# Gyeeta/gyeeta

Measured on AMD Instinct MI355X. Metric: events/sec ingested + p50/p99 quantile error vs reference, 1→8 MI355X, higher is better.
Workload: dtype int64; 1 GPU; C3/C4: 10000 hosts x 1000 services, raw 24-B tcp_ipv4_resp_event_t stream, uniform over services, 1 window (ingest + window close) per step; service_keys_total=10000000, multi_level_windows=0, td_pend_cap=1920, td_pend_cap_is_library_default=False, exchange=none, exchange_requested=none, exchange_fallback=False

## Files before the change

gyeeta_amd/capi.py:

```python
import ctypes as C
import os

HERE = os.path.dirname(os.path.abspath(__file__))
LIB_PATH = os.environ.get("GYS_LIB") or os.path.join(HERE, "lib", "libgysketch.so")

OK, ERR_INVAL, ERR_NOMEM, ERR_HIP, ERR_NOTFOUND, ERR_NOT_OWNER, ERR_STATE, ERR_INTERNAL = 0, -1, -2, -3, -4, -5, -6, -7
MAX_BUCKETS, TD_NB, HLL_P, CMS_D, CMS_W, NSTATES, TOPN = 16, 200, 14, 4, 65536, 6, 10
NLEVELS, LEVEL_RING = 4, 10
TD_PEND_CAP = 896
RCCL_UID_BYTES = 128
KINDS = {"RESP_TIME_HASH": 0, "SEMI_LOG_HASH": 1, "SEMI_LOG_HASH_LO": 2, "DURATION_HASH": 3, "HASH_10_5000": 4, "HASH_5_250": 5,
         "HASH_1_3000": 6, "PERCENT_HASH": 7}


class Config(C.Structure):
    _fields_ = [("struct_size", C.c_uint32), ("device", C.c_int32), ("rank", C.c_uint32), ("nranks", C.c_uint32),
                ("max_hosts", C.c_uint32), ("max_services", C.c_uint32), ("max_clusters", C.c_uint32),
                ("enable_tdigest", C.c_uint32), ("svc_hll_p", C.c_uint32), ("resp_path", C.c_uint32),
                ("max_batch_events", C.c_uint64), ("stream", C.c_void_p), ("reduce_arena", C.c_void_p),
                ("reduce_arena_bytes", C.c_uint64), ("enable_levels", C.c_uint32), ("td_buf_values", C.c_uint32),
                ("conn_pair_cms", C.c_uint32), ("td_pend_cap", C.c_uint32), ("svc_hll_levels", C.c_uint32)]


class ListenerInfo(C.Structure):
# ... 210 lines not shown
    "gys_num_services": (C.c_uint32, [vp]),
    "gys_num_hosts": (C.c_uint32, [vp]),
    "gys_lookup_service": (C.c_int, [vp, C.c_uint64, u32p]),
    "gys_export_hist": (C.c_int, [vp, C.c_int, C.c_uint32, C.c_uint32, vp]),
    "gys_export_conn_bitmap": (C.c_int, [vp, C.c_uint32, C.c_uint32, vp]),
    "gys_export_hll": (C.c_int, [vp, vp]),
    "gys_export_cms": (C.c_int, [vp, C.c_int, vp]),
    "gys_export_tdigest": (C.c_int, [vp, C.c_uint32, C.c_uint32, vp, vp, vp]),
    "gys_export_tdigest_pending": (C.c_int, [vp, C.c_uint32, C.c_uint32, vp, vp]),
    "gys_export_svc_counters": (C.c_int, [vp, C.c_uint32, C.c_uint32, vp]),
    "gys_export_global_hist": (C.c_int, [vp, C.POINTER(HistRec)]),
    "gys_export_svc_hll": (C.c_int, [vp, C.c_uint32, C.c_uint32, vp]),
    "gys_export_svc_hll_level": (C.c_int, [vp, C.c_int, C.c_uint64, C.c_uint32, C.c_uint32, vp]),
    "gys_get_counters": (C.c_int, [vp, C.POINTER(Counters)]),
    "gys_resp_queue_pending": (C.c_int, [vp, u64p]),
    "gys_hist_init_dev": (C.c_int, [vp, C.c_int, vp, C.c_uint32]),
    "gys_hist_add_dev": (C.c_int, [vp, C.c_int, vp, C.c_uint32, vp, vp, C.c_uint64]),
    "gys_hist_merge_dev": (C.c_int, [vp, vp, vp, C.c_uint32]),
    "gys_hist_percentiles_dev": (C.c_int, [vp, C.c_int, vp, C.c_uint32, f32p, C.c_uint32, vp]),
    "gys_profile_enable": (C.c_int, [vp, C.c_int]),
    "gys_profile_reset": (C.c_int, [vp]),
    "gys_profile_get": (C.c_int, [vp, C.c_char_p, f64p, u64p]),
    "gys_profile_names": (C.c_int, [vp, C.c_char_p, C.c_size_t]),
    "gys_debug_read_events_dev": (C.c_int, [vp, vp, C.c_uint64]),
    "gys_gen_resp_events_dev": (C.c_int, [vp, vp, C.c_uint64, C.c_uint64, C.c_uint32, C.c_uint32, C.c_uint32, C.c_uint32, C.POINTER(RespSeg)]),
}

_lib = None


# ... 31 lines not shown
```

gyeeta_amd/csrc/gys_device.hpp:

```cpp
#pragma once

#include <hip/hip_runtime.h>
#include <stdint.h>

#include "../../include/gysketch.h"
#include "../../include/gys_tdigest_tbl.h"

#define GYS_WAVE 64
#ifndef GYS_OPAQUE_VGPR
#define GYS_OPAQUE_VGPR(x) asm volatile("" : "+v"(x))
#endif
#ifndef GYS_DYN_LDS
#define GYS_DYN_LDS(type, name) extern __shared__ type name[]
#endif
#define GYS_SEED 0xceedfeadu
#define GYS_GOLDEN 0x9e3779b9u
#define GYS_NOSLOT 0xFFFFFFFFu
#define GYS_EMPTY_KEY 0xFFFFFFFFFFFFFFFFull

#ifndef GYS_KERNARG
#define GYS_KERNARG 1
#endif
#if GYS_KERNARG && defined(__HIP_DEVICE_COMPILE__)
#define GYS_KERNARG_REF(T, name, arg)                                                             \
// ... 79 lines not shown
	b += (uint32_t)(key >> 32);
	a += (uint32_t)(key & 0xFFFFFFFFu);
	jmix(a, b, c);
	return c;
}

__host__ __device__ __forceinline__ uint32_t host_tbl_hash(uint32_t netns, uint32_t port)
{
	uint32_t x = netns ^ ((port & 0xFFFFu) * 0x9E3779u);
	x ^= x >> 16;
	return x * 0x85EBCA6Bu;
}
__host__ __device__ __forceinline__ uint32_t host_tbl_hash(uint64_t key48) { return host_tbl_hash((uint32_t)(key48 >> 16), (uint32_t)(key48 & 0xFFFFu)); }
__host__ __device__ __forceinline__ uint32_t host_tbl_slot(uint32_t hk, uint32_t mask) { return (hk ^ (hk >> 13)) & mask; }
__host__ __device__ __forceinline__ uint32_t host_tbl_part(uint32_t hk, uint32_t pmask) { return (hk >> 21) & pmask; }

struct HashDef {
	int32_t nthr;
	int32_t is_fixed_diff;
	int32_t arg_bits, t_bits;
	int64_t thr[14];
	int64_t fd_min, fd_maxp1, fd_diff;
};

#define GYS_HASH_DEFS_INIT                                                                                                  \
	{                                                                                                                   \
		{13, 0, 64, 64, {1, 10, 30, 60, 100, 150, 200, 300, 450, 700, 1000, 3000, 15000}, 0, 0, 0},                      \
		{12, 0, 32, 32, {1, 10, 100, 500, 1000, 5000, 25000, 50000, 100000, 300000, 1000000, 5000000}, 0, 0, 0},      \
		{13, 0, 32, 32, {1, 10, 50, 200, 500, 1000, 3000, 6000, 10000, 15000, 25000, 60000, 150000}, 0, 0, 0},        \
		{13, 0, 32, 32, {1, 10, 25, 50, 125, 400, 1000, 3000, 6000, 10000, 25000, 40000, 65000}, 0, 0, 0},            \
// ... 304 lines not shown
```

gyeeta_amd/csrc/gys_engine.hip:

```cpp
#include <hip/hip_runtime.h>

#include <algorithm>
#include <array>
#include <atomic>
#include <chrono>
#include <cmath>
#include <cstdarg>
#include <cstdio>
#include <cstdlib>
#include <cstring>
#include <deque>
#include <map>
#include <string>
#include <thread>
#include <condition_variable>
#include <mutex>
#include <unordered_map>
#include <unordered_set>
#include <vector>

#include <dlfcn.h>
#include <rccl/rccl.h>

#include "gys_kernels.hpp"
// ... 47 lines not shown
	memcpy(&m.first, id, 8);
	memcpy(&m.second, id + 8, 8);
	return m;
}

struct ProfEntry {
	double total_ms = 0;
	uint64_t launches = 0;
	std::vector<std::pair<hipEvent_t, hipEvent_t>> pending;
};

inline uint64_t align_up(uint64_t v, uint64_t a) { return (v + a - 1) / a * a; }

struct HostListeners {
	std::vector<uint64_t> tbl;
	std::vector<uint32_t> slots;
	std::vector<uint32_t> all_slots;
	std::vector<uint64_t> keys;
	uint32_t tbl_off = 0, tbl_cap = 0, lst_off = 0;
	bool on_device = false;
	bool overflow = false;
	std::vector<HostListeners> sub;
	uint32_t sub_desc = 0;
	struct LAddr {
		uint32_t ip32 = 0;
		uint32_t ip128[4] = {0, 0, 0, 0};
		bool any = true;
	};
	struct ChainEnt {
		uint32_t slot;
// ... 407 lines not shown
		set_err("host belongs to rank %u", gys_shard_of(machine_id, c->cfg.nranks));
		return GYS_ERR_NOT_OWNER;
	}
	return GYS_OK;
}

uint32_t next_pow2(uint64_t v)
{
	uint64_t p = 1;
	while (p < v) p <<= 1;
	return (uint32_t)p;
}

inline uint64_t host_key48(uint32_t netns, uint16_t port) { return ((uint64_t)netns << 16) | (uint64_t)port; }

int64_t host_tbl_find(const HostListeners &hl, uint64_t key48)
{
	if (hl.tbl.empty()) return -1;
	const uint32_t mask = (uint32_t)hl.tbl.size() - 1;
	uint32_t h = host_tbl_slot(host_tbl_hash(key48), mask);
	for (uint32_t probes = 0; probes <= mask; ++probes) {
		const uint64_t e = hl.tbl[h];
		if (e == GYS_HOST_TBL_EMPTY) return -1;
		if ((e >> 16) == key48) return (int64_t)h;
		h = (h + 1) & mask;
	}
	return -1;
}

void host_tbl_put(HostListeners &hl, uint64_t key48, uint32_t local)
{
	const uint32_t mask = (uint32_t)hl.tbl.size() - 1;
	uint32_t h = host_tbl_slot(host_tbl_hash(key48), mask);
	while (hl.tbl[h] != GYS_HOST_TBL_EMPTY) h = (h + 1) & mask;
	hl.tbl[h] = (key48 << 16) | (uint64_t)local;
}

inline uint32_t host_part_of(uint64_t key48, uint32_t nparts) { return host_tbl_part(host_tbl_hash(key48), nparts - 1u); }

#define GYS_HOST_TBL_SPARSE 4096u
inline uint32_t host_tbl_capacity(size_t n)
{
	static const uint32_t sparse = [] { const char *e = getenv("GYS_TBL_SPARSE"); return e ? (uint32_t)atoi(e) : GYS_HOST_TBL_SPARSE; }();
	const uint32_t c4 = next_pow2(std::max<uint64_t>(16, (uint64_t)n * 4));
	return c4 <= sparse ? c4 : std::max<uint32_t>(std::min<uint32_t>(sparse, c4), next_pow2(std::max<uint64_t>(16, (uint64_t)n * 2)));
}

int host_tbl_upload(gys_ctx *c, HostListeners &hl, uint32_t desc, uint32_t part, uint32_t nparts, uint32_t cand_off, bool *ok)
{
	*ok = true;
	if (!hl.on_device || hl.tbl.size() > hl.tbl_cap) {
		if (c->htbl_used + hl.tbl.size() > c->htbl_cap || c->hlst_used + hl.tbl.size() / 2 > c->hlst_cap) {
			*ok = false;
			return GYS_OK;
		}
		hl.tbl_off = (uint32_t)c->htbl_used;
		hl.tbl_cap = (uint32_t)hl.tbl.size();
		c->htbl_used += hl.tbl.size();
		hl.lst_off = (uint32_t)c->hlst_used;
		c->hlst_used += hl.tbl.size() / 2;
		hl.on_device = true;
	}
	HIPCHK(hipMemcpyAsync(c->htbl + hl.tbl_off, hl.tbl.data(), hl.tbl.size() * 8, hipMemcpyHostToDevice, c->stream));
	if (!hl.slots.empty()) HIPCHK(hipMemcpyAsync(c->hlst + hl.lst_off, hl.slots.data(), hl.slots.size() * 4, hipMemcpyHostToDevice, c->stream));
	const HostDesc hd{hl.tbl_off, (uint32_t)hl.tbl.size() - 1, (uint32_t)hl.slots.size(), hl.lst_off, part, nparts - 1u, cand_off, 0u};
	HIPCHK(hipMemcpyAsync(c->hdesc + desc, &hd, sizeof(hd), hipMemcpyHostToDevice, c->stream));
	HIPCHK(hipStreamSynchronize(c->stream));
	return GYS_OK;
}

int host_cands_upload(gys_ctx *c, HostListeners &hl)
{
	if (hl.cands.empty()) return GYS_OK;
	if (hl.cands.size() > hl.cand_cap) {
		const uint64_t want = std::max<uint64_t>(16, next_pow2(hl.cands.size()));
		const uint64_t bound = 4ull * c->cfg.max_services + 64ull * c->cfg.max_hosts;
		if (c->cand_used + want > bound) {
			set_err("listener candidate pool exhausted");
			return GYS_ERR_NOMEM;
		}
// ... 148 lines not shown

void host_rebind_local(HostListeners &hl, uint64_t key48, uint32_t slot, uint32_t new_slot)
{
	if (hl.overflow) return;
	HostListeners &t = hl.sub.empty() ? hl : hl.sub[host_part_of(key48, (uint32_t)hl.sub.size())];
	for (uint32_t l = 0; l < t.slots.size(); ++l)
		if (t.slots[l] == slot && t.keys[l] == key48) {
			t.slots[l] = new_slot;
			return;
		}
}

int host_lst_add(gys_ctx *c, uint32_t host, const gys_listener_info *arr, uint32_t n, uint32_t first_slot)
{
	HostListeners &hl = c->host_lst[host];
	auto new_local = [&](uint64_t key48, uint32_t slot) {
		if (hl.overflow) return false;
		HostListeners *t = hl.sub.empty() ? &hl : &hl.sub[host_part_of(key48, (uint32_t)hl.sub.size())];
		while (t->slots.size() >= GYS_HOST_MAX_LOCAL) {
			if (!host_lst_repartition(c, hl, hl.sub.empty() ? 2u : (uint32_t)hl.sub.size() * 2u)) {
				hl.overflow = true;
				auto take = [&](const HostListeners &s) {
					for (uint32_t l = 0; l < s.keys.size(); ++l)
						if (!hl.chain.count(s.keys[l])) hl.okey[s.keys[l]] = s.slots[l];
				};
				if (hl.sub.empty()) take(hl);
				else for (const HostListeners &s : hl.sub) take(s);
				return false;
			}
			t = &hl.sub[host_part_of(key48, (uint32_t)hl.sub.size())];
		}
		host_tbl_insert(hl, *t, key48, slot);
		return true;
	};
	for (uint32_t i = 0; i < n; ++i) {
		const uint64_t key48 = host_key48(arr[i].netns, arr[i].port);
		const uint32_t slot = first_slot + i;
		const HostListeners::LAddr a = listener_addr(arr[i]);
		auto ch = hl.chain.find(key48);
		if (ch != hl.chain.end()) {
			bool replaced = false;
			for (HostListeners::ChainEnt &e : ch->second) {
				if (e.a.any || laddr_equal(e.a, a)) {
					host_rebind_local(hl, key48, e.slot, slot);
					e.slot = slot;
					e.a = a;
					replaced = true;
// ... 24 lines not shown
			if (hl.overflow && a.any) hl.okey[key48] = slot;
		} else if (!hl.overflow) {
			new_local(key48, slot);
			if (hl.overflow && a.any) hl.okey[key48] = slot;
		} else if (a.any) {
			hl.okey[key48] = slot;
		}
		if (!a.any) {
			hl.okey.erase(key48);
			hl.chain[key48].push_back(HostListeners::ChainEnt{slot, a});
			hl.dirty = true;
		}
	}
	if (hl.dirty) {
		host_rebuild(hl);
		const int rc = host_cands_upload(c, hl);
		if (rc) return rc;
		std::vector<uint64_t> kv;
		for (const auto &cf : hl.cand_first) {
			kv.push_back(listener_key(host, (uint32_t)(cf.first >> 16), (uint16_t)(cf.first & 0xFFFFu)));
			kv.push_back((uint64_t)(GYS_SLOT_GROUP | (hl.cand_off + cf.second)));
		}
		if (!kv.empty()) {
			const uint32_t nk = (uint32_t)(kv.size() / 2);
			const int rs = ensure_staging(c, kv.size() * 8, 0);
			if (rs) return rs;
			HIPCHK(hipMemcpyAsync(c->dev_staging, kv.data(), kv.size() * 8, hipMemcpyHostToDevice, c->stream));
			hipLaunchKernelGGL(k_table_set, dim3((nk + 255) / 256), dim3(256), 0, c->stream, c->lk_tbl, (const uint64_t *)c->dev_staging, nk);
			HIPCHK(hipStreamSynchronize(c->stream));
		}
// ... 3531 lines not shown
	HLL_LEVEL_CHECK(level);
	if (!nslots) return GYS_OK;
	uint8_t *tmp = nullptr;
	HIPCHK(hipMalloc((void **)&tmp, (size_t)nslots << c->cfg.svc_hll_p));
	const int rc = hll_level_view(c, level, tusec, first_slot, nslots, tmp, nullptr);
	hipError_t e = hipSuccess;
	if (rc == GYS_OK) e = hipMemcpyAsync(out, tmp, (size_t)nslots << c->cfg.svc_hll_p, hipMemcpyDeviceToHost, c->stream);
	const hipError_t es = hipStreamSynchronize(c->stream);
	hipFree(tmp);
	if (rc) return rc;
	HIPCHK(e);
	HIPCHK(es);
	return GYS_OK;
} GYS_CATCH_ALL

int gys_get_counters(gys_ctx *c, gys_counters *out)
try {
	GYS_ENTER(c);
	if (!c || !out) return GYS_ERR_INVAL;
	uint64_t v[32];
	static_assert(CTR_NUM <= 31, "counter block (the last word is the sink of k_read_events)");
	HIPCHK(hipMemcpyAsync(v, c->counters, sizeof(v), hipMemcpyDeviceToHost, c->stream));
	HIPCHK(hipStreamSynchronize(c->stream));
#ifdef GYS_RESP_TIMING
	{
		unsigned long long t[16];
		HIPCHK(hipMemcpyFromSymbol(t, HIP_SYMBOL(gys::g_resp_timing), sizeof(t)));
		unsigned long long tot = 0;
		for (int i = 0; i < 12; ++i) tot += t[i];
		static const char *nm[12] = {"loads", "probe2", "probe3+", "kept/atomics", "ghist+hash", "hllq/store", "barrier1", "scan1+b", "scan2+b", "image+b", "prologue", "flush"};
// ... 426 lines not shown
```

gyeeta_amd/csrc/gys_kernels.hpp:

```cpp
#pragma once

#include "gys_device.hpp"

namespace gys {

#define GYS_HUGE_VALUE_BITS 20
#define GYS_HUGE_BINS (1u << GYS_HUGE_VALUE_BITS)
#define GYS_ROW_BITS 6
#define GYS_ROW_MASK 0x3Fu
#define GYS_ROW_V6 0x20u
#define GYS_BM_WORDS 32u
#define GYS_STAGED_WORD(tresp, cli_port) ((uint64_t)(((uint32_t)(tresp) << GYS_ROW_BITS) | ((uint32_t)(cli_port) & 0x1Fu)))
#define GYS_STAGED_WORD_FAM(tresp, cli_port, v6) ((uint32_t)(((uint32_t)(tresp) << GYS_ROW_BITS) | ((v6) ? GYS_ROW_V6 : 0u) | ((uint32_t)(cli_port) & 0x1Fu)))

enum { CTR_RESP_EVENTS = 0, CTR_RESP_DROP_RANGE, CTR_RESP_DROP_NOLISTENER, CTR_CONN_EVENTS, CTR_CONN_UNKNOWN, CTR_LSTATE_RECORDS,
       CTR_LSTATE_MISSED, CTR_LSTATE_ERRORS, CTR_LSTATE_DELETED, CTR_TD_MERGES, CTR_TD_MERGE_VALUES, CTR_ACTCONN_RECORDS, CTR_ACTCONN_REMOTE_LISTEN, CTR_ACTCONN_UNKNOWN,
       CTR_CONN_NEW, CTR_CONN_CLOSED, CTR_CONN_CLOSED_NO_NOTIFY, CTR_CONN_CLI_SIDE, CTR_RESP_RUN_OVERFLOW, CTR_NUM };

__global__ void k_table_insert(DevTable t, const uint64_t *keys, uint32_t first_val, uint32_t n, uint32_t *nfail)
{
	const uint32_t i = blockIdx.x * blockDim.x + threadIdx.x;
	if (i >= n) return;
	const uint64_t key = keys[i];
	uint32_t h = get_uint64_hash(key) & t.mask;
// ... 656 lines not shown
__global__ __launch_bounds__(256) void k_cms_reduce(const uint32_t *partial, uint32_t nch, uint32_t *cms32)
{
	const uint32_t i = blockIdx.x * blockDim.x + threadIdx.x;
	if (i >= GYS_CMS_D * GYS_CMS_W) return;
	uint32_t sum = 0;
	for (uint32_t c = 0; c < nch; ++c) sum += partial[(size_t)c * GYS_CMS_D * GYS_CMS_W + i];
	if (sum) cms32[i] += sum;
}

#ifndef GYS_BUCKET_LUT
#define GYS_BUCKET_LUT 1
#endif
#ifndef GYS_SHIFT_SWITCH
#define GYS_SHIFT_SWITCH 0
#endif
#ifndef GYS_PROBE_XOR
#define GYS_PROBE_XOR 1
#endif
#ifndef GYS_BK_BYTES
#define GYS_BK_BYTES 1
#endif
#ifndef GYS_PARK_INDEX
#define GYS_PARK_INDEX 1
#endif
#ifndef GYS_EV_DMA
#define GYS_EV_DMA 0
#endif
#ifndef GYS_EV_DMA_AHEAD
#define GYS_EV_DMA_AHEAD 1
#endif
#if defined(__HIP_DEVICE_COMPILE__)
#ifndef GYS_EV_DMA_CPOL
#define GYS_EV_DMA_CPOL 0
#endif
#define GYS_DMA16(gptr, ldsptr) __builtin_amdgcn_global_load_lds((const __attribute__((address_space(1))) void *)(gptr), (__attribute__((address_space(3))) void *)(ldsptr), 16, 0, GYS_EV_DMA_CPOL)
#define GYS_DMA_WAIT() asm volatile("s_waitcnt vmcnt(0)" ::: "memory")
#else
#define GYS_DMA16(gptr, ldsptr) memcpy((char *)(ldsptr) + 16u * (threadIdx.x & 63u), (const void *)(gptr), 16)
#define GYS_DMA_WAIT() ((void)0)
#endif
#ifndef GYS_EV_PREFETCH
#define GYS_EV_PREFETCH 0
#endif
#ifndef GYS_FLOOR_QUARTER
#define GYS_FLOOR_QUARTER 1
#endif
#ifndef GYS_HASH_FLAT
#define GYS_HASH_FLAT 1
#endif
#ifndef GYS_PROBE_JOINT
#define GYS_PROBE_JOINT 0
#endif
__device__ __forceinline__ void resp_bucket_lut_init(uint32_t *s_bk, uint32_t tid, uint32_t nthreads)
{
	for (uint32_t i = tid; i < 256u; i += nthreads)
		s_bk[i] = resp_bucket((int64_t)(4u * i)) | (resp_bucket((int64_t)(4u * i + 1u)) << 8) | (resp_bucket((int64_t)(4u * i + 2u)) << 16) |
			  (resp_bucket((int64_t)(4u * i + 3u)) << 24);
}
__device__ __forceinline__ uint32_t resp_bucket_lut(const uint32_t *s_bk, uint32_t tresp)
{
	if (!GYS_BUCKET_LUT) return resp_bucket((int64_t)tresp);
#if GYS_BK_BYTES
	uint32_t bix = tresp & 1023u;
#if defined(__HIP_DEVICE_COMPILE__)
	asm volatile("" : "+v"(bix));
#endif
// ... 1 lines not shown
#else
	const uint32_t lo = (s_bk[(tresp >> 2) & 255u] >> ((tresp & 3u) * 8u)) & 0xFFu;
#endif
	const uint32_t hi = 12u + (tresp > 3000u) + (tresp > 15000u);
	return tresp < 1024u ? lo : hi;
}

struct HostDesc {
	uint32_t tbl_off;
	uint32_t mask;
	uint32_t nlst;
	uint32_t lst_off;
	uint32_t part;
	uint32_t pmask;
	uint32_t cand_off;
	uint32_t pad;
};

#define GYS_HOST_TBL_EMPTY 0xFFFFFFFFFFFFFFFFull
#define GYS_EV_DROPPED 0xFFFFFFFFu
#define GYS_HOST_THREADS 1024
#define GYS_RESP_THREADS(TPT) (((TPT) == 12 || (TPT) == 32) ? 512 : 1024)
#define GYS_RESP_WAVES_PER_SIMD(TPT) ((TPT) == 32 ? 2 : 4)
#define GYS_SPLIT_PART 65536u

#ifdef GYS_RESP_TIMING
__device__ unsigned long long g_resp_timing[16];
#define GYS_TICK(i) do { const unsigned long long t_now__ = (unsigned long long)clock64(); tacc[i] += (uint32_t)(t_now__ - t_prev__); t_prev__ = t_now__; } while (0)
#else
#define GYS_TICK(i) do { } while (0)
#endif
struct RespHostP {
	const uint64_t *ev;
	uint64_t n;
// ... 12 lines not shown
	long long run_delta;
	uint32_t *staged;
	const uint32_t *host_spill;
	uint32_t spill_stamp;
	uint64_t *counters;
	uint8_t *svc_hll;
	uint32_t svc_hll_p;
	unsigned long long *ghist;
	long long *gmax;
	uint32_t lds_tbl_entries;
	uint32_t lds_key_entries;
	FinP fin;
	uint32_t dbg;
};

__host__ __device__ __forceinline__ size_t resp_host_lds_bytes(uint32_t tbl_entries, uint32_t key_entries, uint32_t tile)
{
	return ((size_t)tbl_entries + 2u) * 8u + (size_t)key_entries * 24u + ((size_t)tile + 2u) * 6u;
}

#ifndef GYS_RESP_DBG
#define GYS_RESP_DBG 0
#endif
#ifndef GYS_GH_PER_WAVE
#define GYS_GH_PER_WAVE 0
#endif
#define GYS_GH_STRIDE 17u
#define GYS_HQ_CAP 512u
#define GYS_DST_BIAS 65536ull
#ifndef GYS_OPAQUE_LOADED4
#define GYS_OPAQUE_LOADED4(a) asm volatile("" : "+v"(a[0]), "+v"(a[1]), "+v"(a[2]), "+v"(a[3]))
#endif
#ifndef GYS_EV_NT
// ... 43 lines not shown
	constexpr bool DBG = GYS_RESP_DBG != 0;
	constexpr bool V6 = MODE == 2;
	constexpr uint32_t SW = V6 ? GYS_EV6_WORDS : 3u;
	static_assert(MODE == 0 || TPT != 32, "the register-prefetch form exists for the plain IPv4 instance only");
	GYS_DYN_LDS(uint64_t, s_dyn);
	__shared__ uint32_t s_wsum[T / 64];
	__shared__ uint32_t s_drop[2];
	__shared__ uint32_t s_floor[2];
	__shared__ uint32_t s_fqm[4];
	__shared__ unsigned long long s_gh[16 * GYS_GH_STRIDE];
	__shared__ int32_t s_gmax;
	__shared__ uint32_t s_bk[GYS_BUCKET_LUT ? 256 : 1];
	__shared__ uint32_t s_hq[SPILL ? 1 : GYS_HQ_CAP];
	__shared__ uint32_t s_hqn;
	__shared__ FinWg s_fin;
	__shared__ uint32_t s_park[64];
	if (GYS_BUCKET_LUT && !SPILL) resp_bucket_lut_init(s_bk, threadIdx.x, T);
	const uint32_t Lc = p.lds_key_entries;
	uint64_t *s_tbl = s_dyn;
	uint64_t *s_dst = s_dyn + p.lds_tbl_entries + 2u;
	uint32_t *s_cur = (uint32_t *)(s_dst + Lc);
	uint32_t *s_slot = s_cur + Lc;
	uint32_t *s_ts2 = s_slot + Lc;
	uint32_t *s_val = s_ts2 + 2u * Lc;
	uint16_t *s_key = (uint16_t *)(s_val + TILE + 2u);
	const uint32_t tid = threadIdx.x, lane = tid & 63u, wave = tid >> 6;
	const gys_resp_seg seg = p.segs[blockIdx.x];
	const uint64_t e0 = seg.first_event;
	uint32_t nx = blockIdx.x + 1;
	if (seg.reserved)
		while (nx < p.nsegs && p.segs[nx].reserved && p.segs[nx].host_slot == seg.host_slot && p.segs[nx].first_event == e0) ++nx;
	uint64_t e1 = nx < p.nsegs ? p.segs[nx].first_event : p.n;
	if (e1 > p.n) e1 = p.n;
	if (e1 <= e0) return;
	if (SPILL && p.host_spill[seg.host_slot] != p.spill_stamp) return;
	const HostDesc hd = p.hdesc[seg.reserved ? seg.reserved - 1u : seg.host_slot];
	const uint32_t mask = hd.mask, L = hd.nlst;
	for (uint32_t i = tid; i <= mask; i += T) s_tbl[i] = p.htbl[hd.tbl_off + i];
	for (uint32_t k = tid; k < L; k += T) {
		const uint32_t slot = p.hlst[hd.lst_off + k];
		const uint32_t c = p.td_cur[slot];
		s_slot[k] = slot;
		s_cur[k] = SPILL ? (c & GYS_RESPILL_BIT) : c;
		s_ts2[k] = 0;
		s_ts2[Lc + k] = 0;
	}
	if (tid < 2) s_drop[tid] = 0;
	if (tid < 16u * GYS_GH_STRIDE) s_gh[tid] = 0;
	if (tid == 0) {
		s_hqn = 0;
		s_floor[0] = SPILL ? 0u : 0xFFFFFFFFu;
		s_floor[1] = 0xFFFFFFFFu;
		s_gmax = INT32_MIN;
		s_tbl[mask + 1u] = p.htbl[hd.tbl_off];
		s_val[TILE] = 0;
		s_key[TILE] = 0;
	}
	__syncthreads();
	if (!SPILL) {
		if (e1 - e0 >= 4096u) {
			uint32_t mn = 0xFFFFFFFFu;
			const uint4 *h4 = (const uint4 *)p.hll32;
			for (uint32_t i = tid; i < (1u << GYS_HLL_P) / 4u; i += T) {
				const uint4 v = h4[i];
				mn = min(min(mn, min(v.x, v.y)), min(v.z, v.w));
			}
			mn = wave_min_u32(mn);
			if (lane == 0) atomicMin(&s_floor[0], mn);
		} else if (tid == 0) {
			s_floor[0] = 0;
		}
		__syncthreads();
		if (tid == 0) s_floor[1] = s_floor[0];
// ... 33 lines not shown
			const uint32_t oo = o < lim ? o : 0u;
			n0[u] = base[3u * oo];
			n1[u] = base[3u * oo + 1u];
			n2[u] = base[3u * oo + 2u];
		}
	};
	if (PF) {
		const uint64_t left0 = e1 - e0;
		pf_issue(p.ev + 3u * e0, 0u, left0 < (uint64_t)TILE ? (uint32_t)left0 : TILE);
	}
	GYS_TICK(10);
	for (uint64_t t0 = e0; t0 < e1; t0 += TILE, ++tile_no) {
		GYS_RESP_P_RELOAD();
		uint32_t *const s_ts = s_ts2 + (tile_no & 1u) * Lc;
		if (DMA) __syncthreads();
#if GYS_PARK_INDEX
#if defined(__HIP_DEVICE_COMPILE__)
		typedef uint32_t park_ix_t;
#else
		typedef ptrdiff_t park_ix_t;
#endif
		const park_ix_t park_ix = (park_ix_t)(&s_park[lane] - s_ts);
#endif
		if (!SPILL) hll_floor = (uint32_t)__builtin_amdgcn_readfirstlane((int)s_floor[tile_no & 1u]);
		const uint64_t left = e1 - t0;
		const uint32_t rem = left < (uint64_t)TILE ? (uint32_t)left : TILE;
		const uint64_t *const tb = p.ev + (uint64_t)SW * t0;
		uint32_t wd[TPT], lr[TPT];
#pragma unroll
		for (int u = 0; u < TPT; ++u) {
			wd[u] = GYS_EV_DROPPED;
			lr[u] = 0;
		}
#pragma unroll 1
		for (int g = 0; g < TPT; g += 4) {
			if ((uint32_t)g * T >= rem) break;
			uint64_t w0[4], w1[4], w2[4];
			bool in[4];
// ... 107 lines not shown
					nb = tb + 3u * TILE; nlim = left2 < (uint64_t)TILE ? (uint32_t)left2 : TILE; nfirst = 0;
				}
				if (nb != nullptr && lane < 48u) {
					const uint32_t pu = lane / 12u, pl = lane - 12u * pu;
					const uint32_t ev0 = nfirst + pu * T + (tid & ~63u);
					const uint32_t byte = 24u * ev0 + 128u * pl;
					if (byte + 4u <= 24u * nlim) {
						const char *pa = (const char *)nb + byte;
						asm volatile("global_load_dword %0, %1, off" : "=v"(pf_sink) : "v"(pa) : "memory");
					}
				}
			}
#endif
			uint32_t tresp[4], local[4];
			uint64_t ea[4], eb[4];
			bool ok[4], more[4];
#pragma unroll
			for (int u = 0; u < 4; ++u) {
				const uint32_t netns = (uint32_t)w1[u];
				const uint32_t sport = (uint32_t)bswap16((uint16_t)(w1[u] >> 32));
				tresp[u] = (uint32_t)w2[u] - (uint32_t)(w2[u] >> 32);
				const bool range_ok = tresp[u] <= 1000000u;
				if (in[u] && !range_ok && hd.part == 0u) ndrop_range++;
				const uint32_t hk = host_tbl_hash(netns, sport);
				const bool mine = (hk & (hd.pmask << 21)) == (hd.part << 21);
				ok[u] = in[u] && range_ok && mine;
				const uint32_t h = host_tbl_slot(hk, mask);
				ea[u] = s_tbl[h];
				eb[u] = s_tbl[h + 1u];
			}
#pragma unroll
			for (int u = 0; u < 4; ++u) {
				const uint32_t netns = (uint32_t)w1[u], sport = (uint32_t)bswap16((uint16_t)(w1[u] >> 32));
				const uint32_t alo = (uint32_t)ea[u], ahi = (uint32_t)(ea[u] >> 32), blo = (uint32_t)eb[u], bhi = (uint32_t)(eb[u] >> 32);
#if GYS_PROBE_XOR
				const uint32_t sp16 = sport << 16, xa = alo ^ sp16, xb = blo ^ sp16;
				const bool hit_a = ahi == netns && xa < 0xFFFFu, hit_b = bhi == netns && xb < 0xFFFFu;
				uint32_t l = hit_b ? xb : GYS_NOSLOT;
				l = hit_a ? xa : l;
				local[u] = l;
				more[u] = ok[u] && !hit_a && !hit_b;
#else
				const bool hit_a = ahi == netns && (alo >> 16) == sport, hit_b = bhi == netns && (blo >> 16) == sport;
				const bool end_a = (alo & ahi) == 0xFFFFFFFFu, end_b = (blo & bhi) == 0xFFFFFFFFu;
				uint32_t l = (hit_b && !end_a) ? (blo & 0xFFFFu) : GYS_NOSLOT;
				l = hit_a ? (alo & 0xFFFFu) : l;
				local[u] = l;
				more[u] = ok[u] && !hit_a && !hit_b && !end_a && !end_b;
#endif
			}
#ifdef GYS_RESP_TIMING
			asm volatile("" : "+v"(local[0]), "+v"(local[1]), "+v"(local[2]), "+v"(local[3]));
#endif
			GYS_TICK(1);
#if GYS_PROBE_JOINT
			if (more[0] || more[1] || more[2] || more[3]) {
				uint32_t hh[4];
#pragma unroll
				for (int u = 0; u < 4; ++u)
					hh[u] = (host_tbl_slot(host_tbl_hash((uint32_t)w1[u], (uint32_t)bswap16((uint16_t)(w1[u] >> 32))), mask) + 2u) & mask;
				for (uint32_t probes = 2; probes <= mask; ++probes) {
					uint64_t e[4];
#pragma unroll
					for (int u = 0; u < 4; ++u) e[u] = s_tbl[hh[u]];
#pragma unroll
					for (int u = 0; u < 4; ++u) {
						const uint64_t key48 = ((uint64_t)(uint32_t)w1[u] << 16) | (uint64_t)bswap16((uint16_t)(w1[u] >> 32));
						const bool hit = (e[u] >> 16) == key48 && e[u] != GYS_HOST_TBL_EMPTY;
						if (more[u] && hit) local[u] = (uint32_t)(e[u] & 0xFFFFu);
						more[u] = more[u] && !hit && e[u] != GYS_HOST_TBL_EMPTY;
						hh[u] = more[u] ? ((hh[u] + 1u) & mask) : hh[u];
					}
					if (!(more[0] || more[1] || more[2] || more[3])) break;
				}
			}
#else
#pragma unroll
			for (int u = 0; u < 4; ++u) {
				if (more[u]) {
					const uint64_t key48 = ((uint64_t)(uint32_t)w1[u] << 16) | (uint64_t)bswap16((uint16_t)(w1[u] >> 32));
					uint32_t h = (host_tbl_slot(host_tbl_hash((uint32_t)(key48 >> 16), (uint32_t)(key48 & 0xFFFFu)), mask) + 2u) & mask;
					for (uint32_t probes = 2; probes <= mask; ++probes) {
						const uint64_t e = s_tbl[h];
						if ((e >> 16) == key48) {
							local[u] = (uint32_t)(e & 0xFFFFu);
							break;
						}
						if (e == GYS_HOST_TBL_EMPTY) break;
						h = (h + 1) & mask;
					}
				}
			}
#endif
#ifdef GYS_RESP_TIMING
			asm volatile("" : "+v"(local[0]), "+v"(local[1]), "+v"(local[2]), "+v"(local[3]));
#endif
			GYS_TICK(2);
			if (MODE != 0) {
#pragma unroll
				for (int u = 0; u < 4; ++u) {
					if (ok[u] && local[u] != GYS_NOSLOT && (local[u] & GYS_LOCAL_GROUP)) {
						uint32_t e32, e128[4] = {0u, 0u, 0u, 0u}, lc = 0, sl = 0;
						if (V6) {
							const uint32_t o = (uint32_t)(g + u) * T + tid;
							const uint64_t x0 = tb[GYS_EV6_WORDS * o], x1 = tb[GYS_EV6_WORDS * o + 1u];
							e128[0] = (uint32_t)x0; e128[1] = (uint32_t)(x0 >> 32); e128[2] = (uint32_t)x1; e128[3] = (uint32_t)(x1 >> 32);
							e32 = ip6_embedded_v4(e128);
						} else {
							e32 = (uint32_t)w0[u];
						}
						local[u] = cand_resolve(p.cand + hd.cand_off, local[u] & (GYS_LOCAL_GROUP - 1u), e32, e128, &lc, &sl) ? lc : GYS_NOSLOT;
					}
// ... 16 lines not shown
			}
			uint32_t bk[4], rk12[4];
#pragma unroll
			for (int u = 0; u < 4; ++u) {
				const uint32_t dport = (uint32_t)bswap16((uint16_t)(w1[u] >> 48));
				nwd[u] = kept[u] ? ((tresp[u] << GYS_ROW_BITS) | (V6 ? GYS_ROW_V6 : 0u) | (dport & 0x1Fu)) : GYS_EV_DROPPED;
				bk[u] = 15u;
				if (!SPILL) {
					const uint32_t b = resp_bucket_lut(s_bk, tresp[u]);
					bk[u] = kept[u] ? b : 15u;
				}
			}
			if (SPILL && !(kept[0] || kept[1] || kept[2] || kept[3])) continue;
#pragma unroll
			for (int u = 0; u < 4; ++u) {
#if GYS_PARK_INDEX
				const park_ix_t ci = (kept[u] && !(DBG && (p.dbg & 16u))) ? (park_ix_t)nlr[u] : park_ix;
				rk12[u] = atomicAdd(&s_ts[ci], 1u);
#else
				uint32_t *const cell = (kept[u] && !(DBG && (p.dbg & 16u))) ? &s_ts[nlr[u]] : &s_park[lane];
				rk12[u] = atomicAdd(cell, 1u);
#endif
			}
			GYS_TICK(3);
			if (!SPILL) {
#pragma unroll
				for (int u = 0; u < 4; ++u) {
					if (!(DBG && (p.dbg & 8u))) atomicAdd(&s_gh[(GYS_GH_PER_WAVE ? wave : (lane & 15u)) * GYS_GH_STRIDE + bk[u]], (1ull << 40) | (unsigned long long)tresp[u]);
					wmax = max(wmax, (int32_t)nwd[u]);
				}
				GYS_OPAQUE_LOADED4(w0);
			}
#pragma unroll
			for (int u = 0; u < 4; ++u) {
				const uint32_t saddr = (uint32_t)w0[u], daddr = (uint32_t)(w0[u] >> 32);
				const uint16_t sport = bswap16((uint16_t)(w1[u] >> 32)), dport = bswap16((uint16_t)(w1[u] >> 48));
				hrank[u] = 0;
// ... 3175 lines not shown
```

gyeeta_amd/engine.py:

```python
import ctypes as C

import numpy as np

from . import capi, wire

_TORCH_DTYPES = None


def _torch_dtypes():
    global _TORCH_DTYPES
    if _TORCH_DTYPES is None:
        import torch
        _TORCH_DTYPES = {0: torch.uint8, 1: torch.int32, 2: torch.int64}
    return _TORCH_DTYPES


def allreduce_sections(sections, group=None):
    import torch.distributed as dist
    if not (dist.is_available() and dist.is_initialized()) or dist.get_world_size(group) == 1:
        return
    for t, op in sections:
        dist.all_reduce(t, op=dist.ReduceOp.MAX if op == 0 else dist.ReduceOp.SUM, group=group)


# ... 688 lines not shown
        n = self.num_services() - first if n is None else n
        out = np.zeros((n, 1 << self.cfg.svc_hll_p), dtype=np.uint8)
        capi.check(self.L.gys_export_svc_hll(self.h, first, n, C.c_void_p(out.ctypes.data)))
        return out

    def resp_queue_pending(self):
        out = C.c_uint64()
        capi.check(self.L.gys_resp_queue_pending(self.h, C.byref(out)))
        return out.value

    def counters(self):
        out = capi.Counters()
        capi.check(self.L.gys_get_counters(self.h, C.byref(out)))
        return {n: getattr(out, n) for n, _ in out._fields_}

    def profile(self, on=True):
        capi.check(self.L.gys_profile_enable(self.h, 1 if on else 0))

    def profile_reset(self):
        capi.check(self.L.gys_profile_reset(self.h))

    def profile_get(self):
        buf = C.create_string_buffer(1024)
        capi.check(self.L.gys_profile_names(self.h, buf, 1024))
        out = {}
        for name in filter(None, buf.value.decode().split(",")):
            ms, n = C.c_double(), C.c_uint64()
            self.L.gys_profile_get(self.h, name.encode(), C.byref(ms), C.byref(n))
            out[name] = (ms.value, n.value)
        return out
# ... 7 lines not shown
```

include/gysketch.h:

```cpp
#ifndef GYSKETCH_H
#define GYSKETCH_H

#include <stddef.h>
#include <stdint.h>

#ifdef __cplusplus
extern "C" {
#endif

#define GYS_ABI_VERSION 7

enum {
	GYS_OK = 0,
	GYS_ERR_INVAL = -1,
	GYS_ERR_NOMEM = -2,
	GYS_ERR_HIP = -3,
	GYS_ERR_NOTFOUND = -4,
	GYS_ERR_NOT_OWNER = -5,
	GYS_ERR_STATE = -6,
	GYS_ERR_INTERNAL = -7
};

enum {
	GYS_RESP_TIME_HASH = 0,
// ... 358 lines not shown
	uint64_t resp_batches_host_local, resp_batches_general;
	uint64_t window_graph_launches;
	uint64_t resp_batches_host_split;
	uint64_t td_merges, td_merge_values;
	uint64_t actconn_records, actconn_remote_listen, actconn_unknown_listener;
	uint64_t stage_waits;
	uint64_t resp_calls_queued;
	uint64_t resp_submissions;
	uint64_t conn_new, conn_closed, conn_closed_no_notify, conn_client_side;
	uint64_t resp_tail_flushes;
	uint64_t conn_calls_queued, conn_submissions, lstate_calls_queued, lstate_submissions, rec_tail_flushes;
	uint64_t resp_run_overflow;
} gys_counters;
int gys_get_counters(gys_ctx *ctx, gys_counters *out);
int gys_resp_queue_pending(gys_ctx *ctx, uint64_t *events);

int gys_hist_init_dev(gys_ctx *ctx, int kind, gys_hist_rec *d_hist, uint32_t nkeys);
int gys_hist_add_dev(gys_ctx *ctx, int kind, gys_hist_rec *d_hist, uint32_t nkeys, const uint32_t *d_keyidx, const int32_t *d_vals, uint64_t n);
int gys_hist_merge_dev(gys_ctx *ctx, gys_hist_rec *d_dst, const gys_hist_rec *d_src, uint32_t nkeys);
int gys_hist_percentiles_dev(gys_ctx *ctx, int kind, const gys_hist_rec *d_hist, uint32_t nkeys, const float *pcts, uint32_t npct,
			     int64_t *d_out);

int gys_profile_enable(gys_ctx *ctx, int on);
int gys_profile_reset(gys_ctx *ctx);
int gys_profile_get(gys_ctx *ctx, const char *kernel, double *total_ms, uint64_t *launches);
int gys_profile_names(gys_ctx *ctx, char *buf, size_t buflen);

#define GYS_GEN_SPREAD 0xFFFFFFFFu
int gys_debug_read_events_dev(gys_ctx *ctx, const void *d_ev24, uint64_t nevents);
int gys_gen_resp_events_dev(gys_ctx *ctx, void *d_ev24, uint64_t nevents, uint64_t seed, uint32_t first_host, uint32_t nhosts,
// ... 7 lines not shown
```

Measured before the change: 65.10 billion events/s.

## Replace linear-probe host listener table with two-choice cuckoo hashing

Switches the per-host listener hash table from linear probing to a two-slot cuckoo table with a seeded second hash, so the response kernel resolves every lookup with exactly two LDS reads and no probe loop. The host side rebuilds with new seeds or more partitions when placement fails, and the seed travels in the HostDesc. It also drops the separate park array in favour of an index into the timestamp LDS region. The cost is more complex host-side insertion and possibly more repartitioning, and it adds a diagnostic API.

```diff
diff --git a/gyeeta_amd/capi.py b/gyeeta_amd/capi.py
--- a/gyeeta_amd/capi.py
+++ b/gyeeta_amd/capi.py
@@ -248,6 +248,7 @@
     "gys_export_svc_hll_level": (C.c_int, [vp, C.c_int, C.c_uint64, C.c_uint32, C.c_uint32, vp]),
     "gys_get_counters": (C.c_int, [vp, C.POINTER(Counters)]),
     "gys_resp_queue_pending": (C.c_int, [vp, u64p]),
+    "gys_host_listener_tables": (C.c_int, [vp, vp, u32p]),
     "gys_hist_init_dev": (C.c_int, [vp, C.c_int, vp, C.c_uint32]),
     "gys_hist_add_dev": (C.c_int, [vp, C.c_int, vp, C.c_uint32, vp, vp, C.c_uint64]),
     "gys_hist_merge_dev": (C.c_int, [vp, vp, vp, C.c_uint32]),
diff --git a/gyeeta_amd/csrc/gys_device.hpp b/gyeeta_amd/csrc/gys_device.hpp
--- a/gyeeta_amd/csrc/gys_device.hpp
+++ b/gyeeta_amd/csrc/gys_device.hpp
@@ -117,6 +117,51 @@
 __host__ __device__ __forceinline__ uint32_t host_tbl_hash(uint64_t key48) { return host_tbl_hash((uint32_t)(key48 >> 16), (uint32_t)(key48 & 0xFFFFu)); }
 __host__ __device__ __forceinline__ uint32_t host_tbl_slot(uint32_t hk, uint32_t mask) { return (hk ^ (hk >> 13)) & mask; }
 __host__ __device__ __forceinline__ uint32_t host_tbl_part(uint32_t hk, uint32_t pmask) { return (hk >> 21) & pmask; }
+__host__ __device__ __forceinline__ uint32_t host_tbl_mul(uint32_t seed) { return 0x9E3779B1u + seed * 0x7FEB352Eu; }
+__host__ __device__ __forceinline__ uint32_t host_tbl_shift(uint32_t mask) { return (uint32_t)__builtin_clz(mask); }
+__host__ __device__ __forceinline__ uint32_t host_tbl_slot2(uint32_t hk, uint32_t mul, uint32_t shift) { return (hk * mul) >> shift; }
+
+#define GYS_HOST_TBL_EMPTY 0xFFFFFFFFFFFFFFFFull
+#define GYS_HOST_TBL_KICKS 64u
+#define GYS_HOST_TBL_SEEDS 8u
+inline bool host_tbl_place(uint64_t *tbl, uint32_t mask, uint32_t seed, uint64_t *entry)
+{
+	const uint32_t mul = host_tbl_mul(seed), shift = host_tbl_shift(mask);
+	uint64_t e = *entry;
+	uint32_t avoid = 0xFFFFFFFFu;
+	for (uint32_t kick = 0; kick <= GYS_HOST_TBL_KICKS; ++kick) {
+		const uint32_t hk = host_tbl_hash(e >> 16), h1 = host_tbl_slot(hk, mask), h2 = host_tbl_slot2(hk, mul, shift);
+		if (tbl[h1] == GYS_HOST_TBL_EMPTY) { tbl[h1] = e; return true; }
+		if (tbl[h2] == GYS_HOST_TBL_EMPTY) { tbl[h2] = e; return true; }
+		const uint32_t at = h1 == avoid ? h2 : h1;
+		const uint64_t out = tbl[at];
+		tbl[at] = e;
+		e = out;
+		avoid = at;
+	}
+	*entry = e;
+	return false;
+}
+inline bool host_tbl_build(uint64_t *tbl, uint32_t mask, const uint64_t *entries, size_t n, uint32_t *seed)
+{
+	for (uint32_t tries = 0; tries < GYS_HOST_TBL_SEEDS; ++tries, ++*seed) {
+		for (uint32_t i = 0; i <= mask; ++i) tbl[i] = GYS_HOST_TBL_EMPTY;
+		size_t k = 0;
+		for (; k < n; ++k) {
+			uint64_t e = entries[k];
+			if (!host_tbl_place(tbl, mask, *seed, &e)) break;
+		}
+		if (k == n) return true;
+	}
+	return false;
+}
+inline int64_t host_tbl_lookup(const uint64_t *tbl, uint32_t mask, uint32_t seed, uint64_t key48)
+{
+	const uint32_t hk = host_tbl_hash(key48), h1 = host_tbl_slot(hk, mask), h2 = host_tbl_slot2(hk, host_tbl_mul(seed), host_tbl_shift(mask));
+	if (tbl[h1] != GYS_HOST_TBL_EMPTY && (tbl[h1] >> 16) == key48) return (int64_t)h1;
+	if (tbl[h2] != GYS_HOST_TBL_EMPTY && (tbl[h2] >> 16) == key48) return (int64_t)h2;
+	return -1;
+}
 
 struct HashDef {
 	int32_t nthr;
diff --git a/gyeeta_amd/csrc/gys_engine.hip b/gyeeta_amd/csrc/gys_engine.hip
--- a/gyeeta_amd/csrc/gys_engine.hip
+++ b/gyeeta_amd/csrc/gys_engine.hip
@@ -85,6 +85,8 @@
 
 struct HostListeners {
 	std::vector<uint64_t> tbl;
+	uint32_t seed = 0;
+	bool place_fail = false;
 	std::vector<uint32_t> slots;
 	std::vector<uint32_t> all_slots;
 	std::vector<uint64_t> keys;
@@ -522,31 +524,34 @@
 
 inline uint64_t host_key48(uint32_t netns, uint16_t port) { return ((uint64_t)netns << 16) | (uint64_t)port; }
 
+#define GYS_HOST_TBL_SPARSE 4096u
 int64_t host_tbl_find(const HostListeners &hl, uint64_t key48)
 {
-	if (hl.tbl.empty()) return -1;
+	if (hl.tbl.empty() || hl.place_fail) return -1;
+	return host_tbl_lookup(hl.tbl.data(), (uint32_t)hl.tbl.size() - 1, hl.seed, key48);
+}
+
+void host_tbl_put(HostListeners &hl, uint64_t key48, uint32_t local)
+{
+	if (hl.place_fail) return;
 	const uint32_t mask = (uint32_t)hl.tbl.size() - 1;
-	uint32_t h = host_tbl_slot(host_tbl_hash(key48), mask);
-	for (uint32_t probes = 0; probes <= mask; ++probes) {
-		const uint64_t e = hl.tbl[h];
-		if (e == GYS_HOST_TBL_EMPTY) return -1;
-		if ((e >> 16) == key48) return (int64_t)h;
-		h = (h + 1) & mask;
-	}
-	return -1;
-}
-
-void host_tbl_put(HostListeners &hl, uint64_t key48, uint32_t local)
-{
-	const uint32_t mask = (uint32_t)hl.tbl.size() - 1;
-	uint32_t h = host_tbl_slot(host_tbl_hash(key48), mask);
-	while (hl.tbl[h] != GYS_HOST_TBL_EMPTY) h = (h + 1) & mask;
-	hl.tbl[h] = (key48 << 16) | (uint64_t)local;
+	if (host_tbl_lookup(hl.tbl.data(), mask, hl.seed, key48) >= 0) return;
+	uint64_t e = (key48 << 16) | (uint64_t)local;
+	if (host_tbl_place(hl.tbl.data(), mask, hl.seed, &e)) return;
+	std::vector<uint64_t> all{e};
+	for (const uint64_t x : hl.tbl)
+		if (x != GYS_HOST_TBL_EMPTY) all.push_back(x);
+	hl.seed = 0;
+	hl.place_fail = !host_tbl_build(hl.tbl.data(), mask, all.data(), all.size(), &hl.seed);
+	while (hl.place_fail && hl.tbl.size() < GYS_HOST_TBL_SPARSE) {
+		hl.tbl.assign(hl.tbl.size() * 2, GYS_HOST_TBL_EMPTY);
+		hl.seed = 0;
+		hl.place_fail = !host_tbl_build(hl.tbl.data(), (uint32_t)hl.tbl.size() - 1, all.data(), all.size(), &hl.seed);
+	}
 }
 
 inline uint32_t host_part_of(uint64_t key48, uint32_t nparts) { return host_tbl_part(host_tbl_hash(key48), nparts - 1u); }
 
-#define GYS_HOST_TBL_SPARSE 4096u
 inline uint32_t host_tbl_capacity(size_t n)
 {
 	static const uint32_t sparse = [] { const char *e = getenv("GYS_TBL_SPARSE"); return e ? (uint32_t)atoi(e) : GYS_HOST_TBL_SPARSE; }();
@@ -571,7 +576,7 @@
 	}
 	HIPCHK(hipMemcpyAsync(c->htbl + hl.tbl_off, hl.tbl.data(), hl.tbl.size() * 8, hipMemcpyHostToDevice, c->stream));
 	if (!hl.slots.empty()) HIPCHK(hipMemcpyAsync(c->hlst + hl.lst_off, hl.slots.data(), hl.slots.size() * 4, hipMemcpyHostToDevice, c->stream));
-	const HostDesc hd{hl.tbl_off, (uint32_t)hl.tbl.size() - 1, (uint32_t)hl.slots.size(), hl.lst_off, part, nparts - 1u, cand_off, 0u};
+	const HostDesc hd{hl.tbl_off, (uint32_t)hl.tbl.size() - 1, (uint32_t)hl.slots.size(), hl.lst_off, part, nparts - 1u, cand_off, hl.seed + 1u};
 	HIPCHK(hipMemcpyAsync(c->hdesc + desc, &hd, sizeof(hd), hipMemcpyHostToDevice, c->stream));
 	HIPCHK(hipStreamSynchronize(c->stream));
 	return GYS_OK;
@@ -750,23 +755,33 @@
 int host_lst_add(gys_ctx *c, uint32_t host, const gys_listener_info *arr, uint32_t n, uint32_t first_slot)
 {
 	HostListeners &hl = c->host_lst[host];
+	auto more_parts = [&] {
+		if (host_lst_repartition(c, hl, hl.sub.empty() ? 2u : (uint32_t)hl.sub.size() * 2u)) return true;
+		hl.overflow = true;
+		auto take = [&](const HostListeners &s) {
+			for (uint32_t l = 0; l < s.keys.size(); ++l)
+				if (!hl.chain.count(s.keys[l])) hl.okey[s.keys[l]] = s.slots[l];
+		};
+		if (hl.sub.empty()) take(hl);
+		else for (const HostListeners &s : hl.sub) take(s);
+		return false;
+	};
+	auto unplaced = [&] {
+		if (hl.sub.empty()) return hl.place_fail;
+		for (const HostListeners &s : hl.sub)
+			if (s.place_fail) return true;
+		return false;
+	};
 	auto new_local = [&](uint64_t key48, uint32_t slot) {
 		if (hl.overflow) return false;
 		HostListeners *t = hl.sub.empty() ? &hl : &hl.sub[host_part_of(key48, (uint32_t)hl.sub.size())];
 		while (t->slots.size() >= GYS_HOST_MAX_LOCAL) {
-			if (!host_lst_repartition(c, hl, hl.sub.empty() ? 2u : (uint32_t)hl.sub.size() * 2u)) {
-				hl.overflow = true;
-				auto take = [&](const HostListeners &s) {
-					for (uint32_t l = 0; l < s.keys.size(); ++l)
-						if (!hl.chain.count(s.keys[l])) hl.okey[s.keys[l]] = s.slots[l];
-				};
-				if (hl.sub.empty()) take(hl);
-				else for (const HostListeners &s : hl.sub) take(s);
-				return false;
-			}
+			if (!more_parts()) return false;
 			t = &hl.sub[host_part_of(key48, (uint32_t)hl.sub.size())];
 		}
 		host_tbl_insert(hl, *t, key48, slot);
+		while (unplaced())
+			if (!more_parts()) return false;
 		return true;
 	};
 	for (uint32_t i = 0; i < n; ++i) {
@@ -821,6 +836,10 @@
 	}
 	if (hl.dirty) {
 		host_rebuild(hl);
+		while (!hl.overflow && unplaced()) {
+			more_parts();
+			host_rebuild(hl);
+		}
 		const int rc = host_cands_upload(c, hl);
 		if (rc) return rc;
 		std::vector<uint64_t> kv;
@@ -4382,6 +4401,28 @@
 	return GYS_OK;
 } GYS_CATCH_ALL
 
+int gys_host_listener_tables(gys_ctx *c, const uint8_t machine_id[16], uint32_t out[4])
+try {
+	GYS_ENTER(c);
+	if (!c || !machine_id || !out) return GYS_ERR_INVAL;
+	uint32_t host;
+	const int rc = lookup_host(c, machine_id, &host);
+	if (rc) return rc;
+	const HostListeners &hl = c->host_lst[host];
+	out[0] = hl.overflow ? 0u : hl.sub.empty() ? 1u : (uint32_t)hl.sub.size();
+	out[1] = out[2] = out[3] = 0;
+	auto one = [&](const HostListeners &t) {
+		out[1] = std::max(out[1], t.seed);
+		out[2] = std::max(out[2], (uint32_t)t.tbl.size());
+		for (const uint64_t key48 : t.keys)
+			if (host_tbl_find(t, key48) < 0) out[3]++;
+	};
+	if (hl.overflow) return GYS_OK;
+	if (hl.sub.empty()) one(hl);
+	else for (const HostListeners &t : hl.sub) one(t);
+	return GYS_OK;
+} GYS_CATCH_ALL
+
 int gys_get_counters(gys_ctx *c, gys_counters *out)
 try {
 	GYS_ENTER(c);
diff --git a/gyeeta_amd/csrc/gys_kernels.hpp b/gyeeta_amd/csrc/gys_kernels.hpp
--- a/gyeeta_amd/csrc/gys_kernels.hpp
+++ b/gyeeta_amd/csrc/gys_kernels.hpp
@@ -1,4 +1,10 @@
 #pragma once
+#ifndef __HIPCC__
+#include <stdio.h>
+#include <stdlib.h>
+
+#include <vector>
+#endif
 
 #include "gys_device.hpp"
 
@@ -694,14 +700,8 @@
 #ifndef GYS_SHIFT_SWITCH
 #define GYS_SHIFT_SWITCH 0
 #endif
-#ifndef GYS_PROBE_XOR
-#define GYS_PROBE_XOR 1
-#endif
 #ifndef GYS_BK_BYTES
 #define GYS_BK_BYTES 1
-#endif
-#ifndef GYS_PARK_INDEX
-#define GYS_PARK_INDEX 1
 #endif
 #ifndef GYS_EV_DMA
 #define GYS_EV_DMA 0
@@ -727,9 +727,6 @@
 #endif
 #ifndef GYS_HASH_FLAT
 #define GYS_HASH_FLAT 1
-#endif
-#ifndef GYS_PROBE_JOINT
-#define GYS_PROBE_JOINT 0
 #endif
 __device__ __forceinline__ void resp_bucket_lut_init(uint32_t *s_bk, uint32_t tid, uint32_t nthreads)
 {
@@ -761,10 +758,9 @@
 	uint32_t part;
 	uint32_t pmask;
 	uint32_t cand_off;
-	uint32_t pad;
+	uint32_t place;
 };
 
-#define GYS_HOST_TBL_EMPTY 0xFFFFFFFFFFFFFFFFull
 #define GYS_EV_DROPPED 0xFFFFFFFFu
 #define GYS_HOST_THREADS 1024
 #define GYS_RESP_THREADS(TPT) (((TPT) == 12 || (TPT) == 32) ? 512 : 1024)
@@ -807,9 +803,10 @@
 	uint32_t dbg;
 };
 
+#define GYS_RESP_PARK 64u
 __host__ __device__ __forceinline__ size_t resp_host_lds_bytes(uint32_t tbl_entries, uint32_t key_entries, uint32_t tile)
 {
-	return ((size_t)tbl_entries + 2u) * 8u + (size_t)key_entries * 24u + ((size_t)tile + 2u) * 6u;
+	return (size_t)tbl_entries * 8u + (size_t)key_entries * 24u + GYS_RESP_PARK * 4u + ((size_t)tile + 2u) * 6u;
 }
 
 #ifndef GYS_RESP_DBG
@@ -883,15 +880,14 @@
 	__shared__ uint32_t s_hq[SPILL ? 1 : GYS_HQ_CAP];
 	__shared__ uint32_t s_hqn;
 	__shared__ FinWg s_fin;
-	__shared__ uint32_t s_park[64];
 	if (GYS_BUCKET_LUT && !SPILL) resp_bucket_lut_init(s_bk, threadIdx.x, T);
 	const uint32_t Lc = p.lds_key_entries;
 	uint64_t *s_tbl = s_dyn;
-	uint64_t *s_dst = s_dyn + p.lds_tbl_entries + 2u;
+	uint64_t *s_dst = s_dyn + p.lds_tbl_entries;
 	uint32_t *s_cur = (uint32_t *)(s_dst + Lc);
 	uint32_t *s_slot = s_cur + Lc;
 	uint32_t *s_ts2 = s_slot + Lc;
-	uint32_t *s_val = s_ts2 + 2u * Lc;
+	uint32_t *s_val = s_ts2 + 2u * Lc + GYS_RESP_PARK;
 	uint16_t *s_key = (uint16_t *)(s_val + TILE + 2u);
 	const uint32_t tid = threadIdx.x, lane = tid & 63u, wave = tid >> 6;
 	const gys_resp_seg seg = p.segs[blockIdx.x];
@@ -905,6 +901,26 @@
 	if (SPILL && p.host_spill[seg.host_slot] != p.spill_stamp) return;
 	const HostDesc hd = p.hdesc[seg.reserved ? seg.reserved - 1u : seg.host_slot];
 	const uint32_t mask = hd.mask, L = hd.nlst;
+	uint32_t tbl_seed = hd.place - 1u;
+	const uint32_t tbl_shift = host_tbl_shift(mask);
+#ifndef __HIPCC__
+	__shared__ uint32_t s_tbl_seed;
+	if (hd.place == 0u) {
+		if (tid == 0) {
+			std::vector<uint64_t> ent;
+			for (uint32_t i = 0; i <= mask; ++i)
+				if (p.htbl[hd.tbl_off + i] != GYS_HOST_TBL_EMPTY) ent.push_back(p.htbl[hd.tbl_off + i]);
+			uint32_t seed = 0;
+			bool placed = false;
+			for (int round = 0; round < 64 && !placed; ++round) placed = host_tbl_build(s_tbl, mask, ent.data(), ent.size(), &seed);
+			if (!placed) {
+				printf("FAIL: no seed places the %zu keys of a %u-entry table\n", ent.size(), mask + 1u);
+				abort();
+			}
+			s_tbl_seed = seed;
+		}
+	} else
+#endif
 	for (uint32_t i = tid; i <= mask; i += T) s_tbl[i] = p.htbl[hd.tbl_off + i];
 	for (uint32_t k = tid; k < L; k += T) {
 		const uint32_t slot = p.hlst[hd.lst_off + k];
@@ -921,11 +937,14 @@
 		s_floor[0] = SPILL ? 0u : 0xFFFFFFFFu;
 		s_floor[1] = 0xFFFFFFFFu;
 		s_gmax = INT32_MIN;
-		s_tbl[mask + 1u] = p.htbl[hd.tbl_off];
 		s_val[TILE] = 0;
 		s_key[TILE] = 0;
 	}
 	__syncthreads();
+#ifndef __HIPCC__
+	if (hd.place == 0u) tbl_seed = s_tbl_seed;
+#endif
+	const uint32_t tbl_mul = host_tbl_mul(tbl_seed);
 	if (!SPILL) {
 		if (e1 - e0 >= 4096u) {
 			uint32_t mn = 0xFFFFFFFFu;
@@ -989,14 +1008,7 @@
 		GYS_RESP_P_RELOAD();
 		uint32_t *const s_ts = s_ts2 + (tile_no & 1u) * Lc;
 		if (DMA) __syncthreads();
-#if GYS_PARK_INDEX
-#if defined(__HIP_DEVICE_COMPILE__)
-		typedef uint32_t park_ix_t;
-#else
-		typedef ptrdiff_t park_ix_t;
-#endif
-		const park_ix_t park_ix = (park_ix_t)(&s_park[lane] - s_ts);
-#endif
+		const uint32_t park_ix = 2u * Lc - (tile_no & 1u) * Lc + lane;
 		if (!SPILL) hll_floor = (uint32_t)__builtin_amdgcn_readfirstlane((int)s_floor[tile_no & 1u]);
 		const uint64_t left = e1 - t0;
 		const uint32_t rem = left < (uint64_t)TILE ? (uint32_t)left : TILE;
@@ -1134,7 +1146,7 @@
 #endif
 			uint32_t tresp[4], local[4];
 			uint64_t ea[4], eb[4];
-			bool ok[4], more[4];
+			bool ok[4];
 #pragma unroll
 			for (int u = 0; u < 4; ++u) {
 				const uint32_t netns = (uint32_t)w1[u];
@@ -1145,77 +1157,23 @@
 				const uint32_t hk = host_tbl_hash(netns, sport);
 				const bool mine = (hk & (hd.pmask << 21)) == (hd.part << 21);
 				ok[u] = in[u] && range_ok && mine;
-				const uint32_t h = host_tbl_slot(hk, mask);
-				ea[u] = s_tbl[h];
-				eb[u] = s_tbl[h + 1u];
+				ea[u] = s_tbl[host_tbl_slot(hk, mask)];
+				eb[u] = s_tbl[host_tbl_slot2(hk, tbl_mul, tbl_shift)];
 			}
 #pragma unroll
 			for (int u = 0; u < 4; ++u) {
 				const uint32_t netns = (uint32_t)w1[u], sport = (uint32_t)bswap16((uint16_t)(w1[u] >> 32));
 				const uint32_t alo = (uint32_t)ea[u], ahi = (uint32_t)(ea[u] >> 32), blo = (uint32_t)eb[u], bhi = (uint32_t)(eb[u] >> 32);
-#if GYS_PROBE_XOR
 				const uint32_t sp16 = sport << 16, xa = alo ^ sp16, xb = blo ^ sp16;
 				const bool hit_a = ahi == netns && xa < 0xFFFFu, hit_b = bhi == netns && xb < 0xFFFFu;
 				uint32_t l = hit_b ? xb : GYS_NOSLOT;
 				l = hit_a ? xa : l;
 				local[u] = l;
-				more[u] = ok[u] && !hit_a && !hit_b;
-#else
-				const bool hit_a = ahi == netns && (alo >> 16) == sport, hit_b = bhi == netns && (blo >> 16) == sport;
-				const bool end_a = (alo & ahi) == 0xFFFFFFFFu, end_b = (blo & bhi) == 0xFFFFFFFFu;
-				uint32_t l = (hit_b && !end_a) ? (blo & 0xFFFFu) : GYS_NOSLOT;
-				l = hit_a ? (alo & 0xFFFFu) : l;
-				local[u] = l;
-				more[u] = ok[u] && !hit_a && !hit_b && !end_a && !end_b;
-#endif
 			}
 #ifdef GYS_RESP_TIMING
 			asm volatile("" : "+v"(local[0]), "+v"(local[1]), "+v"(local[2]), "+v"(local[3]));
 #endif
 			GYS_TICK(1);
-#if GYS_PROBE_JOINT
-			if (more[0] || more[1] || more[2] || more[3]) {
-				uint32_t hh[4];
-#pragma unroll
-				for (int u = 0; u < 4; ++u)
-					hh[u] = (host_tbl_slot(host_tbl_hash((uint32_t)w1[u], (uint32_t)bswap16((uint16_t)(w1[u] >> 32))), mask) + 2u) & mask;
-				for (uint32_t probes = 2; probes <= mask; ++probes) {
-					uint64_t e[4];
-#pragma unroll
-					for (int u = 0; u < 4; ++u) e[u] = s_tbl[hh[u]];
-#pragma unroll
-					for (int u = 0; u < 4; ++u) {
-						const uint64_t key48 = ((uint64_t)(uint32_t)w1[u] << 16) | (uint64_t)bswap16((uint16_t)(w1[u] >> 32));
-						const bool hit = (e[u] >> 16) == key48 && e[u] != GYS_HOST_TBL_EMPTY;
-						if (more[u] && hit) local[u] = (uint32_t)(e[u] & 0xFFFFu);
-						more[u] = more[u] && !hit && e[u] != GYS_HOST_TBL_EMPTY;
-						hh[u] = more[u] ? ((hh[u] + 1u) & mask) : hh[u];
-					}
-					if (!(more[0] || more[1] || more[2] || more[3])) break;
-				}
-			}
-#else
-#pragma unroll
-			for (int u = 0; u < 4; ++u) {
-				if (more[u]) {
-					const uint64_t key48 = ((uint64_t)(uint32_t)w1[u] << 16) | (uint64_t)bswap16((uint16_t)(w1[u] >> 32));
-					uint32_t h = (host_tbl_slot(host_tbl_hash((uint32_t)(key48 >> 16), (uint32_t)(key48 & 0xFFFFu)), mask) + 2u) & mask;
-					for (uint32_t probes = 2; probes <= mask; ++probes) {
-						const uint64_t e = s_tbl[h];
-						if ((e >> 16) == key48) {
-							local[u] = (uint32_t)(e & 0xFFFFu);
-							break;
-						}
-						if (e == GYS_HOST_TBL_EMPTY) break;
-						h = (h + 1) & mask;
-					}
-				}
-			}
-#endif
-#ifdef GYS_RESP_TIMING
-			asm volatile("" : "+v"(local[0]), "+v"(local[1]), "+v"(local[2]), "+v"(local[3]));
-#endif
-			GYS_TICK(2);
 			if (MODE != 0) {
 #pragma unroll
 				for (int u = 0; u < 4; ++u) {
@@ -1262,13 +1220,8 @@
 			if (SPILL && !(kept[0] || kept[1] || kept[2] || kept[3])) continue;
 #pragma unroll
 			for (int u = 0; u < 4; ++u) {
-#if GYS_PARK_INDEX
-				const park_ix_t ci = (kept[u] && !(DBG && (p.dbg & 16u))) ? (park_ix_t)nlr[u] : park_ix;
+				const uint32_t ci = (kept[u] && !(DBG && (p.dbg & 16u))) ? nlr[u] : park_ix;
 				rk12[u] = atomicAdd(&s_ts[ci], 1u);
-#else
-				uint32_t *const cell = (kept[u] && !(DBG && (p.dbg & 16u))) ? &s_ts[nlr[u]] : &s_park[lane];
-				rk12[u] = atomicAdd(cell, 1u);
-#endif
 			}
 			GYS_TICK(3);
 			if (!SPILL) {
diff --git a/gyeeta_amd/engine.py b/gyeeta_amd/engine.py
--- a/gyeeta_amd/engine.py
+++ b/gyeeta_amd/engine.py
@@ -726,6 +726,11 @@
         capi.check(self.L.gys_get_counters(self.h, C.byref(out)))
         return {n: getattr(out, n) for n, _ in out._fields_}
 
+    def host_listener_tables(self, machine_id):
+        out = (C.c_uint32 * 4)()
+        capi.check(self.L.gys_host_listener_tables(self.h, mid_buf(machine_id), out))
+        return dict(parts=out[0], seed=out[1], entries=out[2], misplaced=out[3])
+
     def profile(self, on=True):
         capi.check(self.L.gys_profile_enable(self.h, 1 if on else 0))
 
diff --git a/include/gysketch.h b/include/gysketch.h
--- a/include/gysketch.h
+++ b/include/gysketch.h
@@ -396,6 +396,7 @@
 } gys_counters;
 int gys_get_counters(gys_ctx *ctx, gys_counters *out);
 int gys_resp_queue_pending(gys_ctx *ctx, uint64_t *events);
+int gys_host_listener_tables(gys_ctx *ctx, const uint8_t machine_id[16], uint32_t out[4]);
 
 int gys_hist_init_dev(gys_ctx *ctx, int kind, gys_hist_rec *d_hist, uint32_t nkeys);
 int gys_hist_add_dev(gys_ctx *ctx, int kind, gys_hist_rec *d_hist, uint32_t nkeys, const uint32_t *d_keyidx, const int32_t *d_vals, uint64_t n);
```

Result: faster. 66.62 billion events/s, median of 6 (+2.3%).
